# nnaisense/evotorch

Hardware: NVIDIA H100
Metric: PGPE generations/sec at popsize=1Mxdim=10k (Rastrigin, fp32) (higher is better)
Workload: dtype f32

## Files before the change

### evotorch_b200/_native.py

```python

from __future__ import annotations

import ctypes
import os
from ctypes import c_float, c_int, c_int64, c_size_t, c_uint64, c_void_p
from typing import Optional

import torch

_PKG = os.path.dirname(os.path.abspath(__file__))
LIB_PATH = os.path.join(_PKG, "lib", "libevok.so")

_P = c_void_p
_SIGNATURES = {
    "evok_abi_version": (c_int, []),
    "evok_launch_count": (c_uint64, []),
    "evok_error_string": (ctypes.c_char_p, [c_int]),
    "evok_sample_eval": (c_int, [c_int, _P, c_int64, _P, _P, c_int64, c_int64, c_int64, c_int, c_uint64, c_uint64, _P, _P, _P]),
    "evok_eval": (c_int, [c_int, _P, c_int64, c_int64, c_int64, _P, _P]),
    "evok_objective_register": (c_int, [_P, c_size_t, _P, c_int, _P]),
    "evok_objective_load": (c_int, [c_int]),
    "evok_rank_workspace_bytes": (c_size_t, [c_int64]),
    "evok_rank": (c_int, [c_int, _P, c_int64, c_int, _P, _P, _P, c_size_t, _P]),
    "evok_argsort": (c_int, [_P, c_int64, c_int, _P, _P, c_size_t, _P]),
    "evok_sample_batched": (c_int, [_P, c_int64, c_int64, _P, c_int64, _P, c_int64, c_int64, c_int64, c_int64, c_int, c_uint64, c_uint64, _P]),
    "evok_rank_batched": (c_int, [c_int, _P, c_int64, c_int64, c_int, _P, _P, c_size_t, _P]),
    "evok_elite_mask_batched": (c_int, [_P, c_int64, c_int64, c_int64, _P, _P, c_size_t, _P]),
    "evok_weights_adjust_batched": (c_int, [_P, c_int64, c_int64, c_int, _P]),
    "evok_grad_batched_workspace_bytes": (c_size_t, [c_int64, c_int64, c_int64]),
    "evok_grad_batched": (c_int, [c_int, _P, c_int64, c_int64, _P, _P, c_int64, _P, c_int64, c_int64, c_int64, c_int64, c_float, c_float, _P, _P, _P,
                                  c_size_t, _P]),
    "evok_clipup_batched": (c_int, [_P, c_int64, c_int64, _P, _P, _P, _P, _P, _P]),
    "evok_sigma_update_batched": (c_int, [_P, _P, c_int64, c_int64, _P, c_int, _P, _P, _P, _P]),
    "evok_rank_table": (c_int, [_P, c_int64, c_int, _P, _P, _P, c_size_t, _P]),
    "evok_cholesky_workspace_bytes": (c_size_t, [c_int64]),
    "evok_cholesky": (c_int, [_P, c_int64, c_int64, _P, c_int64, _P, c_size_t, _P]),
    "evok_cmaes_row_weights": (c_int, [_P, _P, c_int64, c_int64, c_int64, c_int, _P, _P, _P]),
    "evok_cmaes_vector_update": (c_int, [_P, _P, c_int64, _P, _P, _P, _P, _P, c_int64, _P, c_int, _P, _P, _P]),
    "evok_sample_eval_sq": (c_int, [c_int, _P, c_int64, _P, _P, c_int64, c_int64, c_int64, c_uint64, c_uint64, _P, _P, _P, _P]),
    "evok_sepcma_workspace_bytes": (c_size_t, [c_int64, c_int64]),
    "evok_sepcma_moments": (c_int, [_P, _P, c_int, c_int64, c_int64, c_int64, c_uint64, c_uint64, _P, _P, _P, _P, _P, c_size_t, _P]),
    "evok_sepcma_update": (c_int, [_P, _P, _P, c_int64, _P, _P, _P, _P, _P, _P, _P, _P, _P, _P, c_int64, _P, c_int, c_int64, c_float, c_float, _P,
                                   _P]),
    "evok_weights_adjust": (c_int, [_P, c_int64, c_int, _P]),
    "evok_elite_mask": (c_int, [_P, c_int64, c_int64, _P, _P, c_size_t, _P]),
    "evok_grad_workspace_bytes": (c_size_t, [c_int64, c_int64]),
    "evok_grad": (c_int, [c_int, _P, c_int64, _P, _P, _P, c_int64, c_int64, c_float, c_float, _P, _P, _P, c_size_t, _P]),
    "evok_grad_regen": (c_int, [c_int, _P, _P, _P, c_int64, c_int64, c_int64, c_uint64, c_uint64, _P, c_float, c_float, _P, _P, _P,
                                c_size_t, _P]),
    "evok_grad_hybrid": (c_int, [c_int, _P, c_int64, _P, _P, _P, c_int64, c_int64, c_int64, c_uint64, c_uint64, _P, c_int, c_float, c_float, _P,
                                 _P, _P, c_size_t, _P]),
    "evok_grad_auto_split": (c_int, [c_int64]),
    "evok_grad_power_limit_mw": (c_int64, [c_int]),
    "evok_clipup_step": (c_int, [_P, c_int64, _P, c_float, c_float, c_float, _P, _P, _P]),
    "evok_adam_step": (c_int, [_P, c_int64, _P, _P, c_int64, c_float, c_float, c_float, c_float, _P, _P, _P]),
    "evok_sgd_step": (c_int, [_P, c_int64, _P, c_int, c_float, c_float, _P, _P, _P]),
    "evok_axpy": (c_int, [_P, c_int64, c_float, _P, _P]),
    "evok_sigma_update": (c_int, [_P, _P, c_int64, c_float, c_int, _P, c_float, _P, c_float, _P, c_float, _P]),
    "evok_cem_finalize": (c_int, [_P, _P, _P, c_int64, c_int64, _P, _P, _P]),
    "evok_mlp_parameter_length": (c_int64, [c_int, _P]),
    "evok_mlp_forward": (c_int, [_P, c_int64, _P, c_int64, _P, c_int64, c_int64, c_int, _P, _P, _P]),
    "evok_mlp_forward_prep": (c_int, [_P, c_int64, _P, c_int64, _P, c_int64, c_int64, c_int, _P, _P, _P, _P, _P, c_float, c_float, c_float, _P, _P,
                                      c_size_t, _P]),
    "evok_mlp_forward_shared_supported": (c_int, [c_int, _P]),
    "evok_mlp_forward_shared_workspace_bytes": (c_size_t, [c_int64, c_int64, c_int, _P]),
    "evok_mlp_forward_shared": (c_int, [_P, c_int64, c_int64, _P, c_int64, c_int64, c_int, _P, _P, _P, _P, c_size_t, _P]),
    "evok_gemm_gather_rows": (c_int, [_P, c_int64, c_int64, c_int64, c_int64, _P, c_int64, c_int64, c_int64, c_int64, c_int, _P, c_int64, _P]),
    "evok_gemm_gather_rows_workspace_bytes": (c_size_t, [c_int64, c_int64]),
    "evok_gemm_gather_rows_ws": (c_int, [_P, c_int64, c_int64, c_int64, c_int64, _P, c_int64, c_int64, c_int64, c_int64, c_int, _P, c_int64, c_int, _P, c_size_t, _P]),
    "evok_gemm_workspace_bytes": (c_size_t, [c_int64, c_int64, c_int64]),
    "evok_gemm_nt": (c_int, [_P, c_int64, _P, c_int64, c_int64, c_int64, c_int64, _P, c_int64, _P, c_int64, _P, _P, _P, c_size_t, _P]),
    "evok_gemm_nt_affine": (c_int, [_P, c_int64, _P, c_int64, c_int64, c_int64, c_int64, _P, c_int64, _P, _P, c_int64, _P, _P, c_size_t, _P]),
    "evok_transpose_pair": (c_int, [_P, c_int64, c_int64, c_int64, _P, _P, _P, c_int64, _P]),
    "evok_transpose_scale": (c_int, [_P, c_int64, c_int64, c_int64, _P, _P, c_int64, _P]),
    "evok_peer_alloc": (c_int, [c_size_t, _P, _P]),
    "evok_peer_open": (c_int, [_P, _P]),
    "evok_peer_close": (c_int, [_P]),
    "evok_peer_free": (c_int, [_P]),
    "evok_sample_eval_push": (c_int, [c_int, _P, c_int64, _P, _P, c_int64, c_int64, c_int64, c_int, c_uint64, c_uint64, _P, c_int, c_int, _P, _P,
                                      _P, _P, _P]),
    "evok_peer_push": (c_int, [_P, c_int64, c_int64, c_int, c_int, _P, _P, _P, _P]),
    "evok_peer_wait": (c_int, [_P, c_int, _P, _P, c_uint64, _P]),
    "evok_grad_push": (c_int, [c_int, _P, c_int64, _P, _P, _P, c_int64, c_int64, c_int64, c_uint64, c_uint64, _P, c_float, c_float, c_int, c_int,
                               _P, _P, _P, _P, _P, c_size_t, _P]),
    "evok_rank_sharded": (c_int, [c_int, _P, c_int64, c_int, c_int, c_int, _P, _P, _P, _P, _P, _P, _P, c_uint64, _P, _P, _P, c_size_t, _P]),
# ... 91 lines not shown
```

### evotorch_b200/csrc/evok_grad.cu

```cuda
#include <dlfcn.h>

#include <atomic>
#include <cstdlib>

#include "evok_common.cuh"

#ifndef EVOK_GRAD_TMA_DEFAULT
#define EVOK_GRAD_TMA_DEFAULT 1
#endif

namespace evok {

#ifndef EVOK_GRAD_UNROLL
#define EVOK_GRAD_UNROLL 4
#endif
#ifndef EVOK_GRAD_MINB
#define EVOK_GRAD_MINB 4
#endif
#ifndef EVOK_GRAD_CTAS_PER_SM
#define EVOK_GRAD_CTAS_PER_SM 4
#endif
constexpr int kGradThreads = 256;
constexpr int kGradUnroll = EVOK_GRAD_UNROLL;
constexpr int kMaxResidentCtas = kNumSMs * 8;
// ... 260 lines not shown
__device__ __forceinline__ void mbar_expect_tx(uint64_t* bar, uint32_t bytes) {
  asm volatile("mbarrier.arrive.expect_tx.shared::cta.b64 _, [%0], %1;" ::"r"(smem_u32(bar)), "r"(bytes) : "memory");
}
__device__ __forceinline__ void mbar_arrive(uint64_t* bar) {
  asm volatile("mbarrier.arrive.shared::cta.b64 _, [%0];" ::"r"(smem_u32(bar)) : "memory");
}
__device__ __forceinline__ void mbar_wait(uint64_t* bar, uint32_t parity) {
  asm volatile(
      "{\n"
      ".reg .pred P1;\n"
      "LAB_WAIT:\n"
      "mbarrier.try_wait.parity.shared::cta.b64 P1, [%0], %1;\n"
      "@P1 bra DONE;\n"
      "bra LAB_WAIT;\n"
      "DONE:\n"
      "}" ::"r"(smem_u32(bar)), "r"(parity) : "memory");
}
__device__ __forceinline__ void bulk_load(void* dst_smem, const void* src_gmem, uint32_t bytes, uint64_t* bar) {
  asm volatile("cp.async.bulk.shared::cluster.global.mbarrier::complete_tx::bytes [%0], [%1], %2, [%3];" ::"r"(smem_u32(dst_smem)),
               "l"(src_gmem), "r"(bytes), "r"(smem_u32(bar))
               : "memory");
}

constexpr int kSplitPeriod = 16;
__device__ __forceinline__ uint32_t rebuilt_mask(int split) {
  uint32_t m = 0;
#pragma unroll
  for (int k = 0; k < kSplitPeriod; ++k)
    if ((k + 1) * split / kSplitPeriod > k * split / kSplitPeriod) m |= 1u << k;
  return m;
}
__device__ __forceinline__ bool group_rebuilt(uint32_t mask, int64_t g) { return (mask >> ((int)g & (kSplitPeriod - 1))) & 1u; }

template <bool SYM>
__global__ void __launch_bounds__(kTmaThreads, EVOK_GRAD_TMA_CTAS_PER_SM)
    grad_partial_tma_kernel(int form, const float* __restrict__ X, int64_t ldx, const float* __restrict__ w, const float* __restrict__ mu,
                            const float* __restrict__ sigma, int64_t n_units, int64_t D, int64_t units_per_chunk, int split, uint64_t unit0,
                            const __grid_constant__ PhiloxKey key, const uint32_t* __restrict__ stream_off, float* __restrict__ partial) {
  extern __shared__ __align__(128) unsigned char smem_raw[];
  float* tiles = reinterpret_cast<float*>(smem_raw);
  uint64_t* full = reinterpret_cast<uint64_t*>(smem_raw + (size_t)kTmaStages * kTmaRows * kTmaCols * sizeof(float));
  uint64_t* empty = full + kTmaStages;

  const int tid = threadIdx.x, warp = tid >> 5, lane = tid & 31;
  const int64_t col0 = (int64_t)blockIdx.x * kTmaCols;
  const int64_t width = min((int64_t)kTmaCols, D - col0);
  const int64_t r_begin = (int64_t)blockIdx.y * units_per_chunk;
  const int64_t r_end = min(n_units, r_begin + units_per_chunk);
  const int64_t n_rows = r_end - r_begin;
  const int64_t n_groups = (n_rows + kTmaRows - 1) / kTmaRows;
  const int64_t row_stride = (SYM ? 2 : 1) * ldx;
  const uint32_t mask = rebuilt_mask(split);

  if (tid == 0) {
    for (int s = 0; s < kTmaStages; ++s) {
      mbar_init(&full[s], 1);
      mbar_init(&empty[s], kTmaConsumers / 32);
    }
    asm volatile("fence.mbarrier_init.release.cluster;" ::: "memory");
  }
  __syncthreads();

  if (warp == kTmaConsumers / 32) {
    if (lane == 0) {
      const uint32_t row_bytes = (uint32_t)(width * sizeof(float));
      int64_t t = 0;
      for (int64_t g = 0; g < n_groups; ++g) {
        if (group_rebuilt(mask, g)) continue;
        const int s = (int)(t % kTmaStages);
        const uint32_t use = (uint32_t)(t / kTmaStages);
        ++t;
        if (use > 0) mbar_wait(&empty[s], (use - 1) & 1);
        const int64_t r0 = r_begin + g * kTmaRows;
        const int rows = (int)min((int64_t)kTmaRows, r_end - r0);
        mbar_expect_tx(&full[s], rows * row_bytes);
        float* dst = tiles + (size_t)s * kTmaRows * kTmaCols;
        for (int i = 0; i < rows; ++i) bulk_load(dst + (size_t)i * kTmaCols, X + (r0 + i) * row_stride + col0, row_bytes, &full[s]);
      }
    }
    return;
  }

  const int64_t col = col0 + (int64_t)tid * 4;
  const bool active = col < D;
  const uint32_t sw = key.stream_lo + (stream_off ? __ldg(stream_off) : 0u);
  const int frm = SYM ? EVOK_GRAD_SYMMETRIC : form;
  float m[4], sg[4], c1[4], c0[4];
#pragma unroll
  for (int c = 0; c < 4; ++c) {
    sg[c] = active ? __ldg(sigma + col + c) : 1.0f;
    m[c] = active ? __ldg(mu + col + c) : 0.0f;
    if (frm == EVOK_GRAD_EXP) {
      c1[c] = __fdiv_rn(1.0f, sg[c] * sg[c]);
      c0[c] = 1.0f;
    } else if (frm == EVOK_GRAD_MOMENTS) {
      c1[c] = 1.0f;
      c0[c] = 0.0f;
    } else {
      c1[c] = __fdiv_rn(1.0f, sg[c]);
      c0[c] = sg[c];
    }
  }
  float s1[4] = {0.f, 0.f, 0.f, 0.f}, s2[4] = {0.f, 0.f, 0.f, 0.f};

  int64_t t = 0;
  for (int64_t g = 0; g < n_groups; ++g) {
    const int64_t r0 = r_begin + g * kTmaRows;
    const int rows = (int)min((int64_t)kTmaRows, r_end - r0);
    float a[kTmaRows], b[kTmaRows];
    bool need[kTmaRows];
#pragma unroll
    for (int i = 0; i < kTmaRows; ++i) {
      a[i] = b[i] = 0.0f;
      if (i < rows) {
        if (SYM) {
          const float wp = __ldg(w + 2 * (r0 + i)), wm = __ldg(w + 2 * (r0 + i) + 1);
          a[i] = 0.5f * (wp - wm);
          b[i] = 0.5f * (wp + wm);
        } else {
          a[i] = b[i] = __ldg(w + r0 + i);
        }
      }
      need[i] = a[i] != 0.0f || b[i] != 0.0f;
    }
    if (group_rebuilt(mask, g)) {
      if (active) {
        float x[kTmaRows][4];
#pragma unroll
        for (int i = 0; i < kTmaRows; ++i) {
          float z[4];
          normals4(key, sw, unit0 + (uint64_t)(r0 + i), (uint32_t)(col >> 2), z);
#pragma unroll
          for (int c = 0; c < 4; ++c) x[i][c] = fmaf(sg[c], z[c], m[c]);
        }
#pragma unroll
        for (int i = 0; i < kTmaRows; ++i) {
          if (need[i]) {
#pragma unroll
            for (int c = 0; c < 4; ++c) {
              const float e = x[i][c] - m[c];
              s1[c] = fmaf(a[i], e, s1[c]);
              s2[c] = fmaf(b[i], fmaf(e * e, c1[c], -c0[c]), s2[c]);
            }
          }
        }
      }
      continue;
    }
    const int s = (int)(t % kTmaStages);
    const uint32_t use = (uint32_t)(t / kTmaStages);
    ++t;
    mbar_wait(&full[s], use & 1);
    const float4* tile = reinterpret_cast<const float4*>(tiles + (size_t)s * kTmaRows * kTmaCols) + tid;
    if (active) {
      float4 v4[kTmaRows];
#pragma unroll
      for (int i = 0; i < kTmaRows; ++i) v4[i] = tile[(size_t)i * (kTmaCols / 4)];
#pragma unroll
      for (int i = 0; i < kTmaRows; ++i) {
        if (need[i]) {
          const float4 v = v4[i];
          const float x[4] = {v.x, v.y, v.z, v.w};
#pragma unroll
          for (int c = 0; c < 4; ++c) {
            const float e = x[c] - m[c];
            s1[c] = fmaf(a[i], e, s1[c]);
            s2[c] = fmaf(b[i], fmaf(e * e, c1[c], -c0[c]), s2[c]);
          }
        }
      }
    }
    __syncwarp();
    if (lane == 0) mbar_arrive(&empty[s]);
  }
  if (active) {
    float* p1 = partial + ((int64_t)blockIdx.y * 2 + 0) * D + col;
    float* p2 = partial + ((int64_t)blockIdx.y * 2 + 1) * D + col;
#pragma unroll
    for (int c = 0; c < 4; ++c) {
      p1[c] = s1[c];
      p2[c] = s2[c];
    }
  }
}

struct GradPlan {
  int vec, tx, n_coltiles, n_chunks;
  int64_t units_per_chunk;
};

static GradPlan plan_grad(int64_t n_units, int64_t D, bool vec_ok) {
  GradPlan p;
  p.vec = vec_ok ? 4 : 1;
  const int64_t col_threads = (D + p.vec - 1) / p.vec;
  p.tx = 32;
  while (p.tx < kGradThreads && p.tx < col_threads) p.tx <<= 1;
  p.n_coltiles = (int)((col_threads + p.tx - 1) / p.tx);
  const int ty = kGradThreads / p.tx;
  int64_t chunks = (int64_t)kNumSMs * EVOK_GRAD_CTAS_PER_SM / p.n_coltiles;
  const int64_t max_useful = (n_units + (int64_t)ty * kGradUnroll * 16 - 1) / ((int64_t)ty * kGradUnroll * 16);
  if (chunks > max_useful) chunks = max_useful;
  if (chunks < 1) chunks = 1;
  if (chunks > 65535) chunks = 65535;
  p.units_per_chunk = (n_units + chunks - 1) / chunks;
  p.n_chunks = (int)((n_units + p.units_per_chunk - 1) / p.units_per_chunk);
  if (p.n_chunks < 1) p.n_chunks = 1;
  return p;
}

template <int VEC, bool SYM, bool REGEN, bool SEPW = false>
static void launch_partial(const GradPlan& p, int form, const float* X, int64_t ldx, const float* w, const float* mu, const float* sigma,
                           int64_t n_units, int64_t D, uint64_t unit0, uint64_t seed, uint64_t stream_id, const uint32_t* stream_off, float* partial,
                           cudaStream_t st, int64_t n_items = 1, const GradItems* items = nullptr, const SepWeights* sep = nullptr) {
  dim3 grid(p.n_coltiles, p.n_chunks, (unsigned)n_items);
  const PhiloxKey key = make_philox_key(seed, stream_id);
  const GradItems it = items ? *items : GradItems{0, 0, 0, 0, 0};
  const SepWeights sw = sep ? *sep : SepWeights{nullptr, 0, nullptr};
#define EVOK_LAUNCH_TX(TXV)                                                                                                               \
  grad_partial_kernel<VEC, TXV, SYM, REGEN, SEPW><<<grid, kGradThreads, 0, st>>>(form, X, ldx, w, mu, sigma, n_units, D, p.units_per_chunk, \
                                                                                 unit0, key, stream_off, partial, it, sw)
  switch (p.tx) {
    case 32: EVOK_LAUNCH_TX(32); break;
    case 64: EVOK_LAUNCH_TX(64); break;
    case 128: EVOK_LAUNCH_TX(128); break;
    default: EVOK_LAUNCH_TX(256); break;
  }
#undef EVOK_LAUNCH_TX
}

constexpr int kAutoSplitCapped = 2;
constexpr int kAutoSplitFull = 5;
constexpr int64_t kFullPowerMilliwatts = 550000;

static int auto_split_for_power(int64_t milliwatts) { return milliwatts >= kFullPowerMilliwatts ? kAutoSplitFull : kAutoSplitCapped; }

static int64_t enforced_power_limit_mw(int device) {
  char bus_id[32];
  if (cudaDeviceGetPCIBusId(bus_id, (int)sizeof(bus_id), device) != cudaSuccess) {
    cudaGetLastError();
    return -1;
  }
  void* nvml = dlopen("libnvidia-ml.so.1", RTLD_NOW | RTLD_LOCAL);
  if (!nvml) return -1;
  using init_t = int (*)();
  using by_bus_t = int (*)(const char*, void**);
  using limit_t = int (*)(void*, unsigned int*);
  const auto init = reinterpret_cast<init_t>(dlsym(nvml, "nvmlInit_v2"));
  const auto shutdown = reinterpret_cast<init_t>(dlsym(nvml, "nvmlShutdown"));
  const auto by_bus = reinterpret_cast<by_bus_t>(dlsym(nvml, "nvmlDeviceGetHandleByPciBusId_v2"));
  const auto limit = reinterpret_cast<limit_t>(dlsym(nvml, "nvmlDeviceGetEnforcedPowerLimit"));
  int64_t mw = -1;
  if (init && shutdown && by_bus && limit && init() == 0) {
    void* handle = nullptr;
    unsigned int v = 0;
    if (by_bus(bus_id, &handle) == 0 && limit(handle, &v) == 0) mw = v;
    shutdown();
  }
  dlclose(nvml);
  return mw;
}

static int device_auto_split() {
  constexpr int kMaxDevices = 64;
  static std::atomic<int> resolved[kMaxDevices];
  int device = 0;
  if (cudaGetDevice(&device) != cudaSuccess || device < 0 || device >= kMaxDevices) {
    cudaGetLastError();
    return kAutoSplitCapped;
  }
  int s = resolved[device].load(std::memory_order_relaxed);
  if (s == 0) {
    s = auto_split_for_power(enforced_power_limit_mw(device)) + 1;
    resolved[device].store(s, std::memory_order_relaxed);
  }
  return s - 1;
}

static int grad_impl(int form, const float* X, int64_t ldx, const float* w, const float* mu, const float* sigma, int64_t row0, int64_t n_rows,
                     int64_t D, bool regen, uint64_t seed, uint64_t stream_id, const uint32_t* stream_off, float scale_mu, float scale_sigma, float* out_mu,
                     float* out_sigma, void* ws, size_t ws_bytes, void* stream, const GradPush* push = nullptr, int split = 0) {
  if ((!w && n_rows != 0) || !mu || !sigma || !ws || (!regen && !X) || (!push && (!out_mu || !out_sigma))) return EVOK_E_NULLPTR;
  if (form < EVOK_GRAD_SEPARABLE || form > EVOK_GRAD_MOMENTS) return EVOK_E_BADENUM;
  if (n_rows < 0 || D <= 0 || row0 < 0 || (!regen && ldx < D) || split < -1 || split > kSplitPeriod) return EVOK_E_BADSIZE;
  const bool sym = form == EVOK_GRAD_SYMMETRIC;
  if (sym && ((n_rows & 1) || (row0 & 1))) return EVOK_E_ODDROWS;
  if (ws_bytes < evok_grad_workspace_bytes(n_rows, D)) return EVOK_E_WORKSPACE;
  cudaStream_t st = (cudaStream_t)stream;
  const int64_t n_units = sym ? n_rows / 2 : n_rows;
  const bool vec_ok = regen ? true : ((D % 4 == 0) && (ldx % 4 == 0) && aligned16(X));
  const uint64_t unit0 = (uint64_t)(sym ? row0 / 2 : row0);
  float* partial = (float*)ws;
  if (n_units == 0 && push) return launch_finalize(partial, 0, D, scale_mu, scale_sigma, nullptr, nullptr, push, st);
  if (n_units == 0) {
    cudaMemsetAsync(out_mu, 0, (size_t)D * 4, st);
    cudaMemsetAsync(out_sigma, 0, (size_t)D * 4, st);
    return 0;
  }
  const GradPlan p = plan_grad(n_units, D, vec_ok);
  const char* tma_env = getenv("EVOK_GRAD_TMA");
  const int use_tma = tma_env ? atoi(tma_env) : EVOK_GRAD_TMA_DEFAULT;
  if (use_tma && !regen && vec_ok && form != EVOK_GRAD_MOMENTS && D >= 512 && n_units >= 4096) {
    const int n_coltiles = (int)((D + kTmaCols - 1) / kTmaCols);
    int64_t chunks = (int64_t)kNumSMs * EVOK_GRAD_TMA_CTAS_PER_SM / n_coltiles;
    if (chunks < 1) chunks = 1;
    if (chunks > 65535) chunks = 65535;
    const int64_t upc = (n_units + chunks - 1) / chunks;
    const int n_chunks = (int)((n_units + upc - 1) / upc);
    dim3 grid(n_coltiles, n_chunks);
    const int rebuilt = split < 0 ? device_auto_split() : split;
    const PhiloxKey key = make_philox_key(seed, stream_id);
    auto kernel = sym ? grad_partial_tma_kernel<true> : grad_partial_tma_kernel<false>;
    cudaFuncSetAttribute(kernel, cudaFuncAttributeMaxDynamicSharedMemorySize, (int)kTmaSmemBytes);
    kernel<<<grid, kTmaThreads, kTmaSmemBytes, st>>>(form, X, ldx, w, mu, sigma, n_units, D, upc, rebuilt, unit0, key, stream_off, partial);
    EVOK_CHECK_LAUNCH();
    return launch_finalize(partial, n_chunks, D, scale_mu, scale_sigma, out_mu, out_sigma, push, st);
  }
  if (regen) {
    if (sym) launch_partial<4, true, true>(p, form, X, ldx, w, mu, sigma, n_units, D, unit0, seed, stream_id, stream_off, partial, st);
    else launch_partial<4, false, true>(p, form, X, ldx, w, mu, sigma, n_units, D, unit0, seed, stream_id, stream_off, partial, st);
  } else if (vec_ok) {
    if (sym) launch_partial<4, true, false>(p, form, X, ldx, w, mu, sigma, n_units, D, unit0, seed, stream_id, stream_off, partial, st);
    else launch_partial<4, false, false>(p, form, X, ldx, w, mu, sigma, n_units, D, unit0, seed, stream_id, stream_off, partial, st);
  } else {
    if (sym) launch_partial<1, true, false>(p, form, X, ldx, w, mu, sigma, n_units, D, unit0, seed, stream_id, stream_off, partial, st);
    else launch_partial<1, false, false>(p, form, X, ldx, w, mu, sigma, n_units, D, unit0, seed, stream_id, stream_off, partial, st);
  }
  EVOK_CHECK_LAUNCH();
  return launch_finalize(partial, p.n_chunks, D, scale_mu, scale_sigma, out_mu, out_sigma, push, st);
}

}

using namespace evok;

extern "C" EVOK_API size_t evok_grad_workspace_bytes(int64_t n_rows, int64_t D) {
  (void)n_rows;
  if (D <= 0) return 256;
  return ((size_t)kMaxResidentCtas * 1024 + 2 * (size_t)D + 64) * sizeof(float);
}

extern "C" EVOK_API int evok_grad(int form, const float* X, int64_t ldx, const float* w, const float* mu, const float* sigma, int64_t n_rows,
                         int64_t D, float scale_mu, float scale_sigma, float* out_mu, float* out_sigma, void* ws, size_t ws_bytes,
                         void* stream) {
  return grad_impl(form, X, ldx, w, mu, sigma, 0, n_rows, D, false, 0, 0, nullptr, scale_mu, scale_sigma, out_mu, out_sigma, ws, ws_bytes, stream);
}

extern "C" EVOK_API int evok_grad_regen(int form, const float* w, const float* mu, const float* sigma, int64_t row0, int64_t n_rows, int64_t D,
                               uint64_t seed, uint64_t stream_id, const uint32_t* stream_offset_dev, float scale_mu, float scale_sigma,
                               float* out_mu, float* out_sigma, void* ws, size_t ws_bytes, void* stream) {
  return grad_impl(form, nullptr, 0, w, mu, sigma, row0, n_rows, D, true, seed, stream_id, stream_offset_dev, scale_mu, scale_sigma, out_mu, out_sigma, ws,
                   ws_bytes, stream);
}

extern "C" EVOK_API int evok_grad_hybrid(int form, const float* X, int64_t ldx, const float* w, const float* mu, const float* sigma, int64_t row0,
                                         int64_t n_rows, int64_t D, uint64_t seed, uint64_t stream_id, const uint32_t* stream_offset_dev, int split,
                                         float scale_mu, float scale_sigma, float* out_mu, float* out_sigma, void* ws, size_t ws_bytes, void* stream) {
  return grad_impl(form, X, ldx, w, mu, sigma, row0, n_rows, D, false, seed, stream_id, stream_offset_dev, scale_mu, scale_sigma, out_mu, out_sigma, ws,
                   ws_bytes, stream, nullptr, split);
}

extern "C" EVOK_API int evok_grad_auto_split(int64_t power_limit_mw) { return auto_split_for_power(power_limit_mw); }

extern "C" EVOK_API int64_t evok_grad_power_limit_mw(int device) { return enforced_power_limit_mw(device); }

extern "C" EVOK_API size_t evok_sepcma_workspace_bytes(int64_t n_rows, int64_t D) {
  return evok_grad_workspace_bytes(n_rows, D) + (size_t)kMaxResidentCtas * sizeof(float);
}

extern "C" EVOK_API int evok_sepcma_moments(const float* aw, const float* q, int active, int64_t row0, int64_t n_rows, int64_t D, uint64_t seed,
                                            uint64_t stream_id, const uint32_t* stream_offset_dev, float* local, float* S2, float* wsum, void* ws,
                                            size_t ws_bytes, void* stream) {
  if (!aw || (active && !q) || !local || !S2 || !wsum || !ws) return EVOK_E_NULLPTR;
  if (n_rows <= 0 || D <= 0 || row0 < 0) return EVOK_E_BADSIZE;
  if (ws_bytes < evok_sepcma_workspace_bytes(n_rows, D)) return EVOK_E_WORKSPACE;
  cudaStream_t st = (cudaStream_t)stream;
  const GradPlan p = plan_grad(n_rows, D, true);
  float* partial = (float*)ws;
  const SepWeights sep{q, active, partial + evok_grad_workspace_bytes(n_rows, D) / sizeof(float)};
  launch_partial<4, false, true, true>(p, EVOK_GRAD_MOMENTS, nullptr, 0, aw, nullptr, nullptr, n_rows, D, (uint64_t)row0, seed, stream_id,
                                       stream_offset_dev, partial, st, 1, nullptr, &sep);
  EVOK_CHECK_LAUNCH();
  grad_finalize_kernel<true><<<(unsigned)((D + 255) / 256), 256, 0, st>>>(partial, p.n_chunks, D, 1.0f, 1.0f, local, S2, 0, sep.wsum_partial, wsum);
  EVOK_CHECK_LAUNCH();
  return 0;
}

extern "C" EVOK_API int evok_grad_push(int form, const float* X, int64_t ldx, const float* w, const float* mu, const float* sigma, int64_t row0,
                                       int64_t n_rows, int64_t D, uint64_t seed, uint64_t stream_id, const uint32_t* stream_offset_dev,
                                       float scale_mu, float scale_sigma, int world, int rank, void* const* peer_slots, void* const* peer_flags,
                                       const uint64_t* epoch_dev, uint32_t* done_dev, void* ws, size_t ws_bytes, void* stream) {
  if (!peer_slots || !peer_flags || !epoch_dev || !done_dev) return EVOK_E_NULLPTR;
  if (world < 1 || world > EVOK_MAX_PEERS || rank < 0 || rank >= world) return EVOK_E_BADSIZE;
  GradPush push{};
  push.sink.world = world;
// ... 65 lines not shown
```

### evotorch_b200/ops.py

```python

from __future__ import annotations

import ctypes
import math
from typing import Optional

import torch

from . import _native as nat
from .tools.readonlytensor import as_plain_tensor

OBJ_NONE, OBJ_SPHERE, OBJ_RASTRIGIN, OBJ_ACKLEY = 0, 1, 2, 3
OBJ_USER_BASE = 64
OBJECTIVE_IDS = {"sphere": OBJ_SPHERE, "rastrigin": OBJ_RASTRIGIN, "ackley": OBJ_ACKLEY}
RANK_IDS = {"centered": 0, "linear": 1, "nes": 2, "normalized": 3, "raw": 4}
GRAD_SEPARABLE, GRAD_SYMMETRIC, GRAD_EXP, GRAD_MOMENTS = 0, 1, 2, 3
NAN = float("nan")


_timers: Optional[dict] = None


def enable_timers() -> None:
    global _timers
# ... 325 lines not shown
    return mask


def grad(form: int, X: torch.Tensor, w: torch.Tensor, mu: torch.Tensor, sigma: torch.Tensor, scale_mu: float, scale_sigma: float,
         out_mu: Optional[torch.Tensor] = None, out_sigma: Optional[torch.Tensor] = None) -> tuple:
    _mat(X, "samples")
    n, D = X.shape
    _vec(w, "weights", n); _vec(mu, "mu", D); _vec(sigma, "sigma", D)
    out_mu, out_sigma = _out_pair(mu, out_mu, out_sigma)
    ws = nat.workspace(X.device, nat.lib().evok_grad_workspace_bytes(n, D), "grad")
    with _timed("grad"):
        rc = nat.lib().evok_grad(form, X.data_ptr(), X.stride(0), w.data_ptr(), mu.data_ptr(), sigma.data_ptr(), n, D, scale_mu,
                                 scale_sigma, out_mu.data_ptr(), out_sigma.data_ptr(), ws.data_ptr(), ws.numel(), nat.stream_of(X))
    nat.check(rc, "evok_grad")
    return out_mu, out_sigma


def grad_regen(form: int, w: torch.Tensor, mu: torch.Tensor, sigma: torch.Tensor, *, seed: int, stream_id: int, row0: int,
               scale_mu: float, scale_sigma: float, out_mu: Optional[torch.Tensor] = None,
               out_sigma: Optional[torch.Tensor] = None, stream_offset: Optional[torch.Tensor] = None) -> tuple:
    n, D = w.numel(), mu.numel()
    _vec(w, "weights"); _vec(mu, "mu"); _vec(sigma, "sigma", D)
    out_mu, out_sigma = _out_pair(mu, out_mu, out_sigma)
    ws = nat.workspace(mu.device, nat.lib().evok_grad_workspace_bytes(n, D), "grad")
    with _timed("grad_regen"):
        rc = nat.lib().evok_grad_regen(form, w.data_ptr(), mu.data_ptr(), sigma.data_ptr(), row0, n, D, seed, stream_id,
                                       _offset_ptr(stream_offset), scale_mu, scale_sigma, out_mu.data_ptr(), out_sigma.data_ptr(),
                                       ws.data_ptr(), ws.numel(), nat.stream_of(mu))
    nat.check(rc, "evok_grad_regen")
    return out_mu, out_sigma


GRAD_SPLIT_PERIOD = 16


def grad_hybrid(form: int, X: torch.Tensor, w: torch.Tensor, mu: torch.Tensor, sigma: torch.Tensor, *, seed: int, stream_id: int, row0: int,
                scale_mu: float, scale_sigma: float, split: int = -1, out_mu: Optional[torch.Tensor] = None,
                out_sigma: Optional[torch.Tensor] = None, stream_offset: Optional[torch.Tensor] = None) -> tuple:
    _mat(X, "samples")
    n, D = X.shape
    _vec(w, "weights", n); _vec(mu, "mu", D); _vec(sigma, "sigma", D)
    if not -1 <= split <= GRAD_SPLIT_PERIOD:
        raise ValueError(f"split: expected -1 .. {GRAD_SPLIT_PERIOD}, got {split}")
    out_mu, out_sigma = _out_pair(mu, out_mu, out_sigma)
    ws = nat.workspace(X.device, nat.lib().evok_grad_workspace_bytes(n, D), "grad")
    with _timed("grad_hybrid"):
        rc = nat.lib().evok_grad_hybrid(form, X.data_ptr(), X.stride(0), w.data_ptr(), mu.data_ptr(), sigma.data_ptr(), row0, n, D,
                                        seed, stream_id, _offset_ptr(stream_offset), int(split), scale_mu, scale_sigma,
                                        out_mu.data_ptr(), out_sigma.data_ptr(), ws.data_ptr(), ws.numel(), nat.stream_of(X))
    nat.check(rc, "evok_grad_hybrid")
    return out_mu, out_sigma


def clipup_step(g: torch.Tensor, velocity: torch.Tensor, stepsize: float, momentum: float, max_speed: float,
                step_out: Optional[torch.Tensor] = None, mu: Optional[torch.Tensor] = None) -> None:
    D = g.numel()
    _vec(g, "g"); _vec(velocity, "velocity", D)
    with _timed("mu_step"):
        rc = nat.lib().evok_clipup_step(g.data_ptr(), D, velocity.data_ptr(), stepsize, momentum, max_speed, nat.ptr(step_out),
                                        nat.ptr(mu), nat.stream_of(g))
    nat.check(rc, "evok_clipup_step")


def adam_step(g: torch.Tensor, m: torch.Tensor, v: torch.Tensor, t: int, lr: float, beta1: float, beta2: float, eps: float,
              step_out: Optional[torch.Tensor] = None, mu: Optional[torch.Tensor] = None) -> None:
    D = g.numel()
    _vec(g, "g"); _vec(m, "m", D); _vec(v, "v", D)
    rc = nat.lib().evok_adam_step(g.data_ptr(), D, m.data_ptr(), v.data_ptr(), t, lr, beta1, beta2, eps, nat.ptr(step_out), nat.ptr(mu),
                                  nat.stream_of(g))
    nat.check(rc, "evok_adam_step")


def sgd_step(g: torch.Tensor, buf: Optional[torch.Tensor], first_step: bool, lr: float, momentum: float,
             step_out: Optional[torch.Tensor] = None, mu: Optional[torch.Tensor] = None) -> None:
    D = g.numel()
    _vec(g, "g")
    rc = nat.lib().evok_sgd_step(g.data_ptr(), D, nat.ptr(buf), int(first_step), lr, momentum, nat.ptr(step_out), nat.ptr(mu),
                                 nat.stream_of(g))
    nat.check(rc, "evok_sgd_step")


def axpy_(mu: torch.Tensor, g: torch.Tensor, lr: float) -> None:
    D = g.numel()
# ... 290 lines not shown
```

### include/evok.h

```cpp
#ifndef EVOK_H_
#define EVOK_H_

#ifndef __CUDACC_RTC__
#include <stddef.h>
#include <stdint.h>
#endif

#ifdef __cplusplus
extern "C" {
#endif

#define EVOK_ABI_VERSION 1

#if defined(__GNUC__)
#define EVOK_API __attribute__((visibility("default")))
#else
#define EVOK_API
#endif

#define EVOK_E_NULLPTR (-1)
#define EVOK_E_BADSIZE (-2)
#define EVOK_E_BADENUM (-3)
#define EVOK_E_WORKSPACE (-4)
#define EVOK_E_ODDROWS (-5)
// ... 36 lines not shown
#define EVOK_OBJ_KERNEL_SQ 16
#define EVOK_OBJ_KERNEL_EVAL 20
#define EVOK_OBJ_KERNELS 22
int evok_objective_register(const void* cubin, size_t bytes, const char* const* kernel_names_host, int n_kernels, int* id_out_host);
int evok_objective_load(int objective);

size_t evok_rank_workspace_bytes(int64_t N);
int evok_rank(int method, const float* f, int64_t N, int higher_is_better, float* w, int64_t* perm, void* ws,
              size_t ws_bytes, void* stream);

int evok_argsort(const float* keys, int64_t N, int descending, int64_t* perm, void* ws, size_t ws_bytes,
                 void* stream);

int evok_rank_table(const float* keys, int64_t N, int descending, const float* table, float* out, void* ws, size_t ws_bytes, void* stream);

int evok_weights_adjust(float* w, int64_t N, int mode, void* stream);

int evok_elite_mask(const float* w, int64_t N, int64_t num_elites, float* mask, void* ws, size_t ws_bytes,
                    void* stream);

size_t evok_grad_workspace_bytes(int64_t n_rows, int64_t D);
int evok_grad(int form, const float* X, int64_t ldx, const float* w, const float* mu, const float* sigma,
              int64_t n_rows, int64_t D, float scale_mu, float scale_sigma, float* out_mu, float* out_sigma,
              void* ws, size_t ws_bytes, void* stream);

int evok_grad_regen(int form, const float* w, const float* mu, const float* sigma, int64_t row0, int64_t n_rows,
                    int64_t D, uint64_t seed, uint64_t stream_id, const uint32_t* stream_offset_dev, float scale_mu,
                    float scale_sigma, float* out_mu, float* out_sigma, void* ws, size_t ws_bytes, void* stream);

int evok_grad_hybrid(int form, const float* X, int64_t ldx, const float* w, const float* mu, const float* sigma, int64_t row0,
                     int64_t n_rows, int64_t D, uint64_t seed, uint64_t stream_id, const uint32_t* stream_offset_dev, int split,
                     float scale_mu, float scale_sigma, float* out_mu, float* out_sigma, void* ws, size_t ws_bytes, void* stream);

int evok_grad_auto_split(int64_t power_limit_mw);

int64_t evok_grad_power_limit_mw(int device);

int evok_clipup_step(const float* g, int64_t D, float* velocity, float stepsize, float momentum, float max_speed,
                     float* step_out, float* mu, void* stream);
int evok_adam_step(const float* g, int64_t D, float* m, float* v, int64_t t, float lr, float beta1, float beta2,
                   float eps, float* step_out, float* mu, void* stream);
int evok_sgd_step(const float* g, int64_t D, float* buf, int first_step, float lr, float momentum, float* step_out,
                  float* mu, void* stream);
int evok_axpy(const float* g, int64_t D, float lr, float* mu, void* stream);

int evok_sigma_update(float* sigma, const float* g, int64_t D, float lr, int exp_form, const float* lb_vec,
                      float lb, const float* ub_vec, float ub, const float* mc_vec, float mc, void* stream);

int evok_cem_finalize(const float* s1, const float* s2, const float* sigma, int64_t D, int64_t num_elites,
                      float* grad_mu, float* grad_sigma, void* stream);

#define EVOK_ACT_NONE 0
#define EVOK_ACT_TANH 1
#define EVOK_ACT_RELU 2
#define EVOK_ACT_SIGMOID 3
int64_t evok_mlp_parameter_length(int n_layers, const int32_t* dims_host);
int evok_mlp_forward(const float* params, int64_t ldp, const float* obs, int64_t ldo, float* out, int64_t ldout, int64_t N,
                     int n_layers, const int32_t* dims_host, const int32_t* acts_host, void* stream);

int evok_mlp_forward_prep(const float* params, int64_t ldp, const float* obs, int64_t ldo, float* out, int64_t ldout, int64_t N,
                          int n_layers, const int32_t* dims_host, const int32_t* acts_host, const float* obs_sum, const float* obs_sumsq,
                          const int64_t* obs_count_dev, float min_variance, float clip_lo, float clip_hi, const uint8_t* active,
                          void* ws, size_t ws_bytes, void* stream);

int evok_mlp_forward_shared_supported(int n_layers, const int32_t* dims_host);
size_t evok_mlp_forward_shared_workspace_bytes(int64_t N, int64_t B, int n_layers, const int32_t* dims_host);
int evok_mlp_forward_shared(const float* params, int64_t ldp, int64_t N, const float* X, int64_t ldx, int64_t B, int n_layers,
// ... 79 lines not shown
```

Before: 55.26.

## Add per-warp column-slice regeneration to hybrid grad kernel and batch weight loads

Adds a 'cols' parameter so that in each streamed row group a rotating subset of consumer-warp column slices rebuilds samples from Philox instead of loading them, and the TMA producer skips the bytes for those slices. This trades memory traffic for recompute at a finer, per-slice granularity than the existing whole-group split. It also replaces per-row weight __ldg calls with one coalesced warp load per batch of groups, distributed by shuffles. The auto default for cols is 0, so the slicing path mostly stays off and only the weight-batching change affects the default run.

Result: no change. 55.62, median of 6 (+0.6%).

```diff
diff --git a/evotorch_b200/_native.py b/evotorch_b200/_native.py
--- a/evotorch_b200/_native.py
+++ b/evotorch_b200/_native.py
@@ -50,7 +50,10 @@
                                 c_size_t, _P]),
     "evok_grad_hybrid": (c_int, [c_int, _P, c_int64, _P, _P, _P, c_int64, c_int64, c_int64, c_uint64, c_uint64, _P, c_int, c_float, c_float, _P,
                                  _P, _P, c_size_t, _P]),
+    "evok_grad_hybrid_cols": (c_int, [c_int, _P, c_int64, _P, _P, _P, c_int64, c_int64, c_int64, c_uint64, c_uint64, _P, c_int, c_int, c_float,
+                                      c_float, _P, _P, _P, c_size_t, _P]),
     "evok_grad_auto_split": (c_int, [c_int64]),
+    "evok_grad_auto_cols": (c_int, [c_int64]),
     "evok_grad_power_limit_mw": (c_int64, [c_int]),
     "evok_clipup_step": (c_int, [_P, c_int64, _P, c_float, c_float, c_float, _P, _P, _P]),
     "evok_adam_step": (c_int, [_P, c_int64, _P, _P, c_int64, c_float, c_float, c_float, c_float, _P, _P, _P]),
diff --git a/evotorch_b200/csrc/evok_grad.cu b/evotorch_b200/csrc/evok_grad.cu
--- a/evotorch_b200/csrc/evok_grad.cu
+++ b/evotorch_b200/csrc/evok_grad.cu
@@ -316,11 +316,15 @@
 }
 __device__ __forceinline__ bool group_rebuilt(uint32_t mask, int64_t g) { return (mask >> ((int)g & (kSplitPeriod - 1))) & 1u; }
 
+constexpr int kSlices = kTmaConsumers / 32;
+constexpr int kSliceCols = kTmaCols / kSlices;
+
 template <bool SYM>
 __global__ void __launch_bounds__(kTmaThreads, EVOK_GRAD_TMA_CTAS_PER_SM)
     grad_partial_tma_kernel(int form, const float* __restrict__ X, int64_t ldx, const float* __restrict__ w, const float* __restrict__ mu,
-                            const float* __restrict__ sigma, int64_t n_units, int64_t D, int64_t units_per_chunk, int split, uint64_t unit0,
-                            const __grid_constant__ PhiloxKey key, const uint32_t* __restrict__ stream_off, float* __restrict__ partial) {
+                            const float* __restrict__ sigma, int64_t n_units, int64_t D, int64_t units_per_chunk, int split, int cols,
+                            uint64_t unit0, const __grid_constant__ PhiloxKey key, const uint32_t* __restrict__ stream_off,
+                            float* __restrict__ partial) {
   extern __shared__ __align__(128) unsigned char smem_raw[];
   float* tiles = reinterpret_cast<float*>(smem_raw);
   uint64_t* full = reinterpret_cast<uint64_t*>(smem_raw + (size_t)kTmaStages * kTmaRows * kTmaCols * sizeof(float));
@@ -328,13 +332,14 @@
 
   const int tid = threadIdx.x, warp = tid >> 5, lane = tid & 31;
   const int64_t col0 = (int64_t)blockIdx.x * kTmaCols;
-  const int64_t width = min((int64_t)kTmaCols, D - col0);
+  const int width = (int)min((int64_t)kTmaCols, D - col0);
   const int64_t r_begin = (int64_t)blockIdx.y * units_per_chunk;
   const int64_t r_end = min(n_units, r_begin + units_per_chunk);
   const int64_t n_rows = r_end - r_begin;
   const int64_t n_groups = (n_rows + kTmaRows - 1) / kTmaRows;
   const int64_t row_stride = (SYM ? 2 : 1) * ldx;
-  const uint32_t mask = rebuilt_mask(split);
+  const int n_slices = (width + kSliceCols - 1) / kSliceCols;
+  const uint32_t mask = cols < n_slices ? rebuilt_mask(split) : (1u << kSplitPeriod) - 1;
 
   if (tid == 0) {
     for (int s = 0; s < kTmaStages; ++s) {
@@ -347,19 +352,34 @@
 
   if (warp == kTmaConsumers / 32) {
     if (lane == 0) {
-      const uint32_t row_bytes = (uint32_t)(width * sizeof(float));
       int64_t t = 0;
+      int first = 0;
       for (int64_t g = 0; g < n_groups; ++g) {
         if (group_rebuilt(mask, g)) continue;
         const int s = (int)(t % kTmaStages);
         const uint32_t use = (uint32_t)(t / kTmaStages);
         ++t;
+        const int last = first + cols;
+        int lo0 = 0, hi0 = first * kSliceCols, lo1 = last * kSliceCols, hi1 = width;
+        if (last > n_slices) {
+          lo0 = (last - n_slices) * kSliceCols;
+          hi0 = first * kSliceCols;
+          lo1 = hi1 = 0;
+        }
+        hi0 = min(hi0, width);
+        lo1 = min(lo1, width);
+        first = last >= n_slices ? last - n_slices : last;
         if (use > 0) mbar_wait(&empty[s], (use - 1) & 1);
         const int64_t r0 = r_begin + g * kTmaRows;
         const int rows = (int)min((int64_t)kTmaRows, r_end - r0);
-        mbar_expect_tx(&full[s], rows * row_bytes);
+        const uint32_t bytes0 = (uint32_t)(hi0 - lo0) * sizeof(float), bytes1 = (uint32_t)(hi1 - lo1) * sizeof(float);
+        mbar_expect_tx(&full[s], rows * (bytes0 + bytes1));
         float* dst = tiles + (size_t)s * kTmaRows * kTmaCols;
-        for (int i = 0; i < rows; ++i) bulk_load(dst + (size_t)i * kTmaCols, X + (r0 + i) * row_stride + col0, row_bytes, &full[s]);
+        for (int i = 0; i < rows; ++i) {
+          const float* src = X + (r0 + i) * row_stride + col0;
+          if (bytes0) bulk_load(dst + (size_t)i * kTmaCols + lo0, src + lo0, bytes0, &full[s]);
+          if (bytes1) bulk_load(dst + (size_t)i * kTmaCols + lo1, src + lo1, bytes1, &full[s]);
+        }
       }
     }
     return;
@@ -387,75 +407,98 @@
   }
   float s1[4] = {0.f, 0.f, 0.f, 0.f}, s2[4] = {0.f, 0.f, 0.f, 0.f};
 
+  constexpr int kWeightsPerUnit = SYM ? 2 : 1;
+  constexpr int kBatchGroups = 32 / (kWeightsPerUnit * kTmaRows);
+  const int64_t w_end = r_end * kWeightsPerUnit;
+  auto load_batch = [&](int64_t g) {
+    const int64_t k = (r_begin + g * kTmaRows) * kWeightsPerUnit + lane;
+    return k < w_end ? __ldg(w + k) : 0.0f;
+  };
+  float w_cur = load_batch(0), w_next = load_batch(kBatchGroups);
+
   int64_t t = 0;
+  int first = 0;
+  int gb = 0;
   for (int64_t g = 0; g < n_groups; ++g) {
     const int64_t r0 = r_begin + g * kTmaRows;
-    const int rows = (int)min((int64_t)kTmaRows, r_end - r0);
+    if (gb == kBatchGroups) {
+      gb = 0;
+      w_cur = w_next;
+      w_next = load_batch(g + kBatchGroups);
+    }
     float a[kTmaRows], b[kTmaRows];
     bool need[kTmaRows];
 #pragma unroll
     for (int i = 0; i < kTmaRows; ++i) {
-      a[i] = b[i] = 0.0f;
-      if (i < rows) {
-        if (SYM) {
-          const float wp = __ldg(w + 2 * (r0 + i)), wm = __ldg(w + 2 * (r0 + i) + 1);
-          a[i] = 0.5f * (wp - wm);
-          b[i] = 0.5f * (wp + wm);
-        } else {
-          a[i] = b[i] = __ldg(w + r0 + i);
-        }
+      const int k = (gb * kTmaRows + i) * kWeightsPerUnit;
+      if (SYM) {
+        const float wp = __shfl_sync(0xffffffffu, w_cur, k), wm = __shfl_sync(0xffffffffu, w_cur, k + 1);
+        a[i] = 0.5f * (wp - wm);
+        b[i] = 0.5f * (wp + wm);
+      } else {
+        a[i] = b[i] = __shfl_sync(0xffffffffu, w_cur, k);
       }
       need[i] = a[i] != 0.0f || b[i] != 0.0f;
     }
-    if (group_rebuilt(mask, g)) {
-      if (active) {
-        float x[kTmaRows][4];
-#pragma unroll
-        for (int i = 0; i < kTmaRows; ++i) {
-          float z[4];
-          normals4(key, sw, unit0 + (uint64_t)(r0 + i), (uint32_t)(col >> 2), z);
-#pragma unroll
-          for (int c = 0; c < 4; ++c) x[i][c] = fmaf(sg[c], z[c], m[c]);
-        }
-#pragma unroll
-        for (int i = 0; i < kTmaRows; ++i) {
-          if (need[i]) {
-#pragma unroll
-            for (int c = 0; c < 4; ++c) {
-              const float e = x[i][c] - m[c];
-              s1[c] = fmaf(a[i], e, s1[c]);
-              s2[c] = fmaf(b[i], fmaf(e * e, c1[c], -c0[c]), s2[c]);
+    ++gb;
+    bool rebuild = group_rebuilt(mask, g);
+    if (!rebuild) {
+      const int s = (int)(t % kTmaStages);
+      const uint32_t use = (uint32_t)(t / kTmaStages);
+      ++t;
+      int d = warp - first;
+      if (d < 0) d += n_slices;
+      rebuild = d < cols;
+      first += cols;
+      if (first >= n_slices) first -= n_slices;
+      mbar_wait(&full[s], use & 1);
+      if (rebuild) {
+        if (lane == 0) mbar_arrive(&empty[s]);
+      } else {
+        const float4* tile = reinterpret_cast<const float4*>(tiles + (size_t)s * kTmaRows * kTmaCols) + tid;
+        if (active) {
+          float4 v4[kTmaRows];
+#pragma unroll
+          for (int i = 0; i < kTmaRows; ++i) v4[i] = tile[(size_t)i * (kTmaCols / 4)];
+#pragma unroll
+          for (int i = 0; i < kTmaRows; ++i) {
+            if (need[i]) {
+              const float4 v = v4[i];
+              const float x[4] = {v.x, v.y, v.z, v.w};
+#pragma unroll
+              for (int c = 0; c < 4; ++c) {
+                const float e = x[c] - m[c];
+                s1[c] = fmaf(a[i], e, s1[c]);
+                s2[c] = fmaf(b[i], fmaf(e * e, c1[c], -c0[c]), s2[c]);
+              }
             }
           }
         }
-      }
-      continue;
-    }
-    const int s = (int)(t % kTmaStages);
-    const uint32_t use = (uint32_t)(t / kTmaStages);
-    ++t;
-    mbar_wait(&full[s], use & 1);
-    const float4* tile = reinterpret_cast<const float4*>(tiles + (size_t)s * kTmaRows * kTmaCols) + tid;
-    if (active) {
-      float4 v4[kTmaRows];
-#pragma unroll
-      for (int i = 0; i < kTmaRows; ++i) v4[i] = tile[(size_t)i * (kTmaCols / 4)];
+        __syncwarp();
+        if (lane == 0) mbar_arrive(&empty[s]);
+      }
+    }
+    if (rebuild && active) {
+      float x[kTmaRows][4];
+#pragma unroll
+      for (int i = 0; i < kTmaRows; ++i) {
+        float z[4];
+        normals4(key, sw, unit0 + (uint64_t)(r0 + i), (uint32_t)(col >> 2), z);
+#pragma unroll
+        for (int c = 0; c < 4; ++c) x[i][c] = fmaf(sg[c], z[c], m[c]);
+      }
 #pragma unroll
       for (int i = 0; i < kTmaRows; ++i) {
         if (need[i]) {
-          const float4 v = v4[i];
-          const float x[4] = {v.x, v.y, v.z, v.w};
 #pragma unroll
           for (int c = 0; c < 4; ++c) {
-            const float e = x[c] - m[c];
+            const float e = x[i][c] - m[c];
             s1[c] = fmaf(a[i], e, s1[c]);
             s2[c] = fmaf(b[i], fmaf(e * e, c1[c], -c0[c]), s2[c]);
           }
         }
       }
     }
-    __syncwarp();
-    if (lane == 0) mbar_arrive(&empty[s]);
   }
   if (active) {
     float* p1 = partial + ((int64_t)blockIdx.y * 2 + 0) * D + col;
@@ -518,6 +561,11 @@
 
 static int auto_split_for_power(int64_t milliwatts) { return milliwatts >= kFullPowerMilliwatts ? kAutoSplitFull : kAutoSplitCapped; }
 
+constexpr int kAutoColsCapped = 0;
+constexpr int kAutoColsFull = 0;
+
+static int auto_cols_for_power(int64_t milliwatts) { return milliwatts >= kFullPowerMilliwatts ? kAutoColsFull : kAutoColsCapped; }
+
 static int64_t enforced_power_limit_mw(int device) {
   char bus_id[32];
   if (cudaDeviceGetPCIBusId(bus_id, (int)sizeof(bus_id), device) != cudaSuccess) {
@@ -544,28 +592,29 @@
   return mw;
 }
 
-static int device_auto_split() {
+static int64_t device_power_limit_mw() {
   constexpr int kMaxDevices = 64;
-  static std::atomic<int> resolved[kMaxDevices];
+  static std::atomic<int64_t> resolved[kMaxDevices];
   int device = 0;
   if (cudaGetDevice(&device) != cudaSuccess || device < 0 || device >= kMaxDevices) {
     cudaGetLastError();
-    return kAutoSplitCapped;
-  }
-  int s = resolved[device].load(std::memory_order_relaxed);
-  if (s == 0) {
-    s = auto_split_for_power(enforced_power_limit_mw(device)) + 1;
-    resolved[device].store(s, std::memory_order_relaxed);
-  }
-  return s - 1;
+    return -1;
+  }
+  int64_t v = resolved[device].load(std::memory_order_relaxed);
+  if (v == 0) {
+    v = enforced_power_limit_mw(device) + 2;
+    resolved[device].store(v, std::memory_order_relaxed);
+  }
+  return v - 2;
 }
 
 static int grad_impl(int form, const float* X, int64_t ldx, const float* w, const float* mu, const float* sigma, int64_t row0, int64_t n_rows,
                      int64_t D, bool regen, uint64_t seed, uint64_t stream_id, const uint32_t* stream_off, float scale_mu, float scale_sigma, float* out_mu,
-                     float* out_sigma, void* ws, size_t ws_bytes, void* stream, const GradPush* push = nullptr, int split = 0) {
+                     float* out_sigma, void* ws, size_t ws_bytes, void* stream, const GradPush* push = nullptr, int split = 0, int cols = 0) {
   if ((!w && n_rows != 0) || !mu || !sigma || !ws || (!regen && !X) || (!push && (!out_mu || !out_sigma))) return EVOK_E_NULLPTR;
   if (form < EVOK_GRAD_SEPARABLE || form > EVOK_GRAD_MOMENTS) return EVOK_E_BADENUM;
-  if (n_rows < 0 || D <= 0 || row0 < 0 || (!regen && ldx < D) || split < -1 || split > kSplitPeriod) return EVOK_E_BADSIZE;
+  if (n_rows < 0 || D <= 0 || row0 < 0 || (!regen && ldx < D) || split < -1 || split > kSplitPeriod || cols < -1 || cols > kSlices)
+    return EVOK_E_BADSIZE;
   const bool sym = form == EVOK_GRAD_SYMMETRIC;
   if (sym && ((n_rows & 1) || (row0 & 1))) return EVOK_E_ODDROWS;
   if (ws_bytes < evok_grad_workspace_bytes(n_rows, D)) return EVOK_E_WORKSPACE;
@@ -591,11 +640,14 @@
     const int64_t upc = (n_units + chunks - 1) / chunks;
     const int n_chunks = (int)((n_units + upc - 1) / upc);
     dim3 grid(n_coltiles, n_chunks);
-    const int rebuilt = split < 0 ? device_auto_split() : split;
+    const int64_t mw = split < 0 || cols < 0 ? device_power_limit_mw() : -1;
+    const int rebuilt = split < 0 ? auto_split_for_power(mw) : split;
+    const int rebuilt_cols = cols < 0 ? auto_cols_for_power(mw) : cols;
     const PhiloxKey key = make_philox_key(seed, stream_id);
     auto kernel = sym ? grad_partial_tma_kernel<true> : grad_partial_tma_kernel<false>;
     cudaFuncSetAttribute(kernel, cudaFuncAttributeMaxDynamicSharedMemorySize, (int)kTmaSmemBytes);
-    kernel<<<grid, kTmaThreads, kTmaSmemBytes, st>>>(form, X, ldx, w, mu, sigma, n_units, D, upc, rebuilt, unit0, key, stream_off, partial);
+    kernel<<<grid, kTmaThreads, kTmaSmemBytes, st>>>(form, X, ldx, w, mu, sigma, n_units, D, upc, rebuilt, rebuilt_cols, unit0, key, stream_off,
+                                                     partial);
     EVOK_CHECK_LAUNCH();
     return launch_finalize(partial, n_chunks, D, scale_mu, scale_sigma, out_mu, out_sigma, push, st);
   }
@@ -639,11 +691,21 @@
 extern "C" EVOK_API int evok_grad_hybrid(int form, const float* X, int64_t ldx, const float* w, const float* mu, const float* sigma, int64_t row0,
                                          int64_t n_rows, int64_t D, uint64_t seed, uint64_t stream_id, const uint32_t* stream_offset_dev, int split,
                                          float scale_mu, float scale_sigma, float* out_mu, float* out_sigma, void* ws, size_t ws_bytes, void* stream) {
+  return evok_grad_hybrid_cols(form, X, ldx, w, mu, sigma, row0, n_rows, D, seed, stream_id, stream_offset_dev, split, -1, scale_mu, scale_sigma,
+                               out_mu, out_sigma, ws, ws_bytes, stream);
+}
+
+extern "C" EVOK_API int evok_grad_hybrid_cols(int form, const float* X, int64_t ldx, const float* w, const float* mu, const float* sigma,
+                                              int64_t row0, int64_t n_rows, int64_t D, uint64_t seed, uint64_t stream_id,
+                                              const uint32_t* stream_offset_dev, int split, int cols, float scale_mu, float scale_sigma,
+                                              float* out_mu, float* out_sigma, void* ws, size_t ws_bytes, void* stream) {
   return grad_impl(form, X, ldx, w, mu, sigma, row0, n_rows, D, false, seed, stream_id, stream_offset_dev, scale_mu, scale_sigma, out_mu, out_sigma, ws,
-                   ws_bytes, stream, nullptr, split);
+                   ws_bytes, stream, nullptr, split, cols);
 }
 
 extern "C" EVOK_API int evok_grad_auto_split(int64_t power_limit_mw) { return auto_split_for_power(power_limit_mw); }
+
+extern "C" EVOK_API int evok_grad_auto_cols(int64_t power_limit_mw) { return auto_cols_for_power(power_limit_mw); }
 
 extern "C" EVOK_API int64_t evok_grad_power_limit_mw(int device) { return enforced_power_limit_mw(device); }
 
diff --git a/evotorch_b200/ops.py b/evotorch_b200/ops.py
--- a/evotorch_b200/ops.py
+++ b/evotorch_b200/ops.py
@@ -381,23 +381,26 @@
 
 
 GRAD_SPLIT_PERIOD = 16
+GRAD_COL_SLICES = 8
 
 
 def grad_hybrid(form: int, X: torch.Tensor, w: torch.Tensor, mu: torch.Tensor, sigma: torch.Tensor, *, seed: int, stream_id: int, row0: int,
-                scale_mu: float, scale_sigma: float, split: int = -1, out_mu: Optional[torch.Tensor] = None,
+                scale_mu: float, scale_sigma: float, split: int = -1, cols: int = -1, out_mu: Optional[torch.Tensor] = None,
                 out_sigma: Optional[torch.Tensor] = None, stream_offset: Optional[torch.Tensor] = None) -> tuple:
     _mat(X, "samples")
     n, D = X.shape
     _vec(w, "weights", n); _vec(mu, "mu", D); _vec(sigma, "sigma", D)
     if not -1 <= split <= GRAD_SPLIT_PERIOD:
         raise ValueError(f"split: expected -1 .. {GRAD_SPLIT_PERIOD}, got {split}")
+    if not -1 <= cols <= GRAD_COL_SLICES:
+        raise ValueError(f"cols: expected -1 .. {GRAD_COL_SLICES}, got {cols}")
     out_mu, out_sigma = _out_pair(mu, out_mu, out_sigma)
     ws = nat.workspace(X.device, nat.lib().evok_grad_workspace_bytes(n, D), "grad")
     with _timed("grad_hybrid"):
-        rc = nat.lib().evok_grad_hybrid(form, X.data_ptr(), X.stride(0), w.data_ptr(), mu.data_ptr(), sigma.data_ptr(), row0, n, D,
-                                        seed, stream_id, _offset_ptr(stream_offset), int(split), scale_mu, scale_sigma,
-                                        out_mu.data_ptr(), out_sigma.data_ptr(), ws.data_ptr(), ws.numel(), nat.stream_of(X))
-    nat.check(rc, "evok_grad_hybrid")
+        rc = nat.lib().evok_grad_hybrid_cols(form, X.data_ptr(), X.stride(0), w.data_ptr(), mu.data_ptr(), sigma.data_ptr(), row0, n, D,
+                                             seed, stream_id, _offset_ptr(stream_offset), int(split), int(cols), scale_mu, scale_sigma,
+                                             out_mu.data_ptr(), out_sigma.data_ptr(), ws.data_ptr(), ws.numel(), nat.stream_of(X))
+    nat.check(rc, "evok_grad_hybrid_cols")
     return out_mu, out_sigma
 
 
diff --git a/include/evok.h b/include/evok.h
--- a/include/evok.h
+++ b/include/evok.h
@@ -92,7 +92,14 @@
                      int64_t n_rows, int64_t D, uint64_t seed, uint64_t stream_id, const uint32_t* stream_offset_dev, int split,
                      float scale_mu, float scale_sigma, float* out_mu, float* out_sigma, void* ws, size_t ws_bytes, void* stream);
 
+int evok_grad_hybrid_cols(int form, const float* X, int64_t ldx, const float* w, const float* mu, const float* sigma, int64_t row0,
+                          int64_t n_rows, int64_t D, uint64_t seed, uint64_t stream_id, const uint32_t* stream_offset_dev, int split,
+                          int cols, float scale_mu, float scale_sigma, float* out_mu, float* out_sigma, void* ws, size_t ws_bytes,
+                          void* stream);
+
 int evok_grad_auto_split(int64_t power_limit_mw);
+
+int evok_grad_auto_cols(int64_t power_limit_mw);
 
 int64_t evok_grad_power_limit_mw(int device);
 
```
